# ygina/sidekick

Measured on AMD Instinct MI355X. Metric: quACK encode identifiers/s (device-resident), u32 ids, threshold t=32, higher is better.
Workload: dtype u32; 1 GPU; encode 1e+09 u32 ids per GPU at t=32, device-resident; ids_per_gpu=1000000000, global_ids=1000000000, threshold=32, bits=32, seed=0x5eed0002, parallelism=shard1, collectives=single

## Files before the change

### sidekick_amd/csrc/api.hip

```cpp
#include <string.h>

#include <algorithm>
#include <chrono>
#include <thread>
#include <vector>

#include "ctx.h"
#include "field.h"

using namespace qk;

#pragma clang diagnostic ignored "-Wunused-value"
#pragma clang diagnostic ignored "-Wunused-result"

namespace qk {

QK_WARM_KERNEL(api)

hipStream_t pick_stream(qk_ctx *ctx, void *stream) {
    (void)ctx;
    return (hipStream_t)stream;
}

int scratch_acquire(qk_ctx *ctx, hipStream_t s) {
// ... 551 lines not shown
    if (!ctx) return QK_E_INVAL;
    std::lock_guard<std::mutex> g(ctx->mu);
    ctx->profiling = on != 0;
    return QK_OK;
}

int qk_ctx_kernel_stats(qk_ctx *ctx, double *total_ms, uint64_t *launches) {
    if (!ctx || !total_ms || !launches) return QK_E_INVAL;
    std::lock_guard<std::mutex> g(ctx->mu);
    double tot = 0;
    uint64_t cnt = 0;
    int rc = QK_OK;
    for (auto &pr : ctx->prof_pending) {
        if (hipEventSynchronize(pr.second) != hipSuccess) rc = QK_E_HIP;
        float ms = 0;
        if (hipEventElapsedTime(&ms, pr.first, pr.second) == hipSuccess) { tot += ms; ++cnt; }
        ctx->ev_pool.push_back(pr.first);
        ctx->ev_pool.push_back(pr.second);
    }
    ctx->prof_pending.clear();
    *total_ms = tot;
    *launches = cnt;
    return rc;
}

int qk_ctx_trim(qk_ctx *ctx) {
    if (!ctx) return QK_E_INVAL;
    std::lock_guard<std::mutex> g(ctx->mu);
    if (ctx->retired.empty()) return QK_OK;
    QK_HIP_TRY(hipSetDevice(ctx->device));
    int rc = QK_OK;
    for (void *r : ctx->retired)
        if (hipFree(r) != hipSuccess) rc = QK_E_HIP;
    ctx->retired.clear();
    return rc;
}

int qk_ctx_set_grid(qk_ctx *ctx, uint32_t blocks) {
    if (!ctx) return QK_E_INVAL;
    ctx->grid_override = blocks;
    return QK_OK;
}

int qk_ctx_set_knob(qk_ctx *ctx, const char *name, int64_t value) {
    if (!ctx || !name) return QK_E_INVAL;
    struct K {
        const char *name;
        int qk_knobs::*field;
        int64_t lo, hi;
    };
    static const K table[] = {
        {"grid_mult", &qk_knobs::grid_mult, 1, 8},
        {"enc_dyn", &qk_knobs::enc_dyn, 0, 1},
        {"u32_basis", &qk_knobs::u32_basis, 0, 1},
        {"flow_hist", &qk_knobs::flow_hist, 0, 1 << 20},
        {"flow_byslot", &qk_knobs::flow_byslot, 0, 2},
        {"root_test", &qk_knobs::root_test, 0, 2},
        {"comm_fault", &qk_knobs::comm_fault, 0, 1 << 20},
        {"comm_delay_ms", &qk_knobs::comm_delay_ms, 0, 600000},
        {"rt_karg", &qk_knobs::rt_karg, 0, 1},
    };
    for (const K &k : table)
        if (strcmp(k.name, name) == 0) {
            if (value < k.lo || value > k.hi) return QK_E_INVAL;
            std::lock_guard<std::mutex> g(ctx->mu);
            ctx->knobs.*(k.field) = (int)value;
            return QK_OK;
        }
    return QK_E_INVAL;
}

__global__ void k_clock_probe(uint64_t *out, uint64_t ticks) {
    const uint64_t c0 = __builtin_amdgcn_s_memtime(), r0 = __builtin_amdgcn_s_memrealtime();
    uint64_t c1, r1;
    do {
        __builtin_amdgcn_s_sleep(32);
        c1 = __builtin_amdgcn_s_memtime();
        r1 = __builtin_amdgcn_s_memrealtime();
    } while (r1 - r0 < ticks);
    if (threadIdx.x == 0) {
        out[0] = c1 - c0;
        out[1] = r1 - r0;
    }
}

int qk_clock_probe(qk_ctx *ctx, uint32_t microseconds, uint64_t *d_out, void *stream) {
    if (!ctx || !d_out || !microseconds || microseconds > 10000000u) return QK_E_INVAL;
    if (!is_device_ptr(d_out)) return QK_E_INVAL;
    QK_HIP_TRY(hipSetDevice(ctx->device));
    hipLaunchKernelGGL(k_clock_probe, dim3(1), dim3(64), 0, (hipStream_t)stream, d_out, (uint64_t)microseconds * 100);
    QK_HIP_TRY(hipGetLastError());
    return QK_OK;
}

int qk_host_alloc(size_t bytes, void **out) {
    if (!out) return QK_E_INVAL;
    if (hipHostMalloc(out, bytes, hipHostMallocDefault) != hipSuccess) { *out = nullptr; return QK_E_NOMEM; }
    return QK_OK;
}
int qk_host_free(void *p) {
    if (p && hipHostFree(p) != hipSuccess) return QK_E_HIP;
    return QK_OK;
}

int qk_u32_encode_device_async(qk_ctx *ctx, const uint32_t *d_ids, size_t n, uint32_t t, uint64_t *d_partial,
                               void *stream) {
    if (!ctx || !d_partial || (n && !d_ids)) return QK_E_INVAL;
// ... 157 lines not shown
```

### sidekick_amd/csrc/bsgs.h

```cpp
#pragma once
#include <hip/hip_runtime.h>
#include <stdint.h>

#include "basis32.h"
#include "field.h"

namespace qk {
namespace bsgs {

constexpr int BLOCK = 256;
constexpr int WAVES = BLOCK / 64;

__device__ __forceinline__ uint64_t shfl_xor_u64(uint64_t v, int m) {
    const uint32_t lo = __shfl_xor((int)(uint32_t)v, m, 64);
    const uint32_t hi = __shfl_xor((int)(uint32_t)(v >> 32), m, 64);
    return ((uint64_t)hi << 32) | lo;
}

#define QK_MAC4V(P0, P1, P2, P3)                                                                       \
    "v_mad_u64_u32 %0, " P0 ", %8, %9, %0\n\t"                                                         \
    "v_mad_u64_u32 %1, " P1 ", %8, %10, %1\n\t"                                                        \
    "v_mad_u64_u32 %2, " P2 ", %8, %11, %2\n\t"                                                        \
    "v_mad_u64_u32 %3, " P3 ", %8, %12, %3\n\t"                                                        \
    "v_addc_co_u32_e64 %4, " P0 ", %4, 0, " P0 "\n\t"                                                  \
    "v_addc_co_u32_e64 %5, " P1 ", %5, 0, " P1 "\n\t"                                                  \
    "v_addc_co_u32_e64 %6, " P2 ", %6, 0, " P2 "\n\t"                                                  \
    "v_addc_co_u32_e64 %7, " P3 ", %7, 0, " P3
#define QK_MAC4S(P0, P1, P2, P3, T)                                                                       \
    "v_mad_u64_u32 %0, " P0 ", %8, %9, %0\n\t"                                                         \
    "v_mad_u64_u32 %1, " P1 ", %8, %10, %1\n\t"                                                        \
    "v_mad_u64_u32 %2, " P2 ", %8, %11, %2\n\t"                                                        \
    "v_mad_u64_u32 %3, " P3 ", %8, %12, %3\n\t"                                                        \
    "s_bcnt1_i32_b64 " T ", " P0 "\n\ts_add_u32 %4, %4, " T "\n\t"                                          \
    "s_bcnt1_i32_b64 " T ", " P1 "\n\ts_add_u32 %5, %5, " T "\n\t"                                          \
    "s_bcnt1_i32_b64 " T ", " P2 "\n\ts_add_u32 %6, %6, " T "\n\t"                                          \
    "s_bcnt1_i32_b64 " T ", " P3 "\n\ts_add_u32 %7, %7, " T
#define QK_ADD4V(P0, P1, P2, P3)                                                                       \
    "v_add_co_u32_e64 %0, " P0 ", %0, %8\n\t"                                                          \
    "v_add_co_u32_e64 %1, " P1 ", %1, %9\n\t"                                                          \
    "v_add_co_u32_e64 %2, " P2 ", %2, %10\n\t"                                                         \
    "v_add_co_u32_e64 %3, " P3 ", %3, %11\n\t"                                                         \
    "v_addc_co_u32_e64 %4, " P0 ", %4, 0, " P0 "\n\t"                                                  \
    "v_addc_co_u32_e64 %5, " P1 ", %5, 0, " P1 "\n\t"                                                  \
    "v_addc_co_u32_e64 %6, " P2 ", %6, 0, " P2 "\n\t"                                                  \
    "v_addc_co_u32_e64 %7, " P3 ", %7, 0, " P3
#define QK_ADD4S(P0, P1, P2, P3, T)                                                                       \
    "v_add_co_u32_e64 %0, " P0 ", %0, %8\n\t"                                                          \
    "v_add_co_u32_e64 %1, " P1 ", %1, %9\n\t"                                                          \
    "v_add_co_u32_e64 %2, " P2 ", %2, %10\n\t"                                                         \
    "v_add_co_u32_e64 %3, " P3 ", %3, %11\n\t"                                                         \
    "s_bcnt1_i32_b64 " T ", " P0 "\n\ts_add_u32 %4, %4, " T "\n\t"                                          \
    "s_bcnt1_i32_b64 " T ", " P1 "\n\ts_add_u32 %5, %5, " T "\n\t"                                          \
    "s_bcnt1_i32_b64 " T ", " P2 "\n\ts_add_u32 %6, %6, " T "\n\t"                                          \
    "s_bcnt1_i32_b64 " T ", " P3 "\n\ts_add_u32 %7, %7, " T
#define QK_SET0 "s[40:41]", "s[42:43]", "s[44:45]", "s[46:47]"
#define QK_SET1 "s[48:49]", "s[50:51]", "s[52:53]", "s[54:55]"
#define QK_SET0T QK_SET0, "s56"
// ... 91 lines not shown
                                      uint32_t b0, uint32_t b1) {
    uint64_t k0, k1;
    asm("v_mad_u64_u32 %0, %4, %6, %7, %0\n\t"
        "v_mad_u64_u32 %1, %5, %6, %8, %1\n\t"
        "s_nop 0\n\t"
        "v_addc_co_u32_e64 %2, %4, %2, 0, %4\n\t"
        "v_addc_co_u32_e64 %3, %5, %3, 0, %5"
        : "+v"(a0), "+v"(a1), "+v"(c0), "+v"(c1), "=&s"(k0), "=&s"(k1)
        : "v"(A), "v"(b0), "v"(b1));
}
__device__ __forceinline__ void add2v(uint32_t &l0, uint32_t &l1, uint32_t &c0, uint32_t &c1, uint32_t b0,
                                      uint32_t b1) {
    uint64_t k0, k1;
    asm("v_add_co_u32_e64 %0, %4, %0, %6\n\t"
        "v_add_co_u32_e64 %1, %5, %1, %7\n\t"
        "s_nop 0\n\t"
        "v_addc_co_u32_e64 %2, %4, %2, 0, %4\n\t"
        "v_addc_co_u32_e64 %3, %5, %3, 0, %5"
        : "+v"(l0), "+v"(l1), "+v"(c0), "+v"(c1), "=&s"(k0), "=&s"(k1)
        : "v"(b0), "v"(b1));
}

#define QK_ROW4M(P0, P1, P2, P3)                                                                       \
    "v_mad_u64_u32 %0, " P0 ", %4, 1, %0\n\t"                                                          \
    "v_mad_u64_u32 %1, " P1 ", %5, 1, %1\n\t"                                                          \
    "v_mad_u64_u32 %2, " P2 ", %6, 1, %2\n\t"                                                          \
    "v_mad_u64_u32 %3, " P3 ", %7, 1, %3"
template <int SET>
__device__ __forceinline__ void row4m(uint64_t &a0, uint64_t &a1, uint64_t &a2, uint64_t &a3, uint32_t b0,
                                      uint32_t b1, uint32_t b2, uint32_t b3) {
    if constexpr (SET == 0)
        asm volatile(QK_EXPAND(QK_ROW4M, QK_SET0)
            : "+v"(a0), "+v"(a1), "+v"(a2), "+v"(a3)
            : "v"(b0), "v"(b1), "v"(b2), "v"(b3)
            : QK_CLOB0);
    else
        asm volatile(QK_EXPAND(QK_ROW4M, QK_SET1)
            : "+v"(a0), "+v"(a1), "+v"(a2), "+v"(a3)
            : "v"(b0), "v"(b1), "v"(b2), "v"(b3)
            : QK_CLOB1);
}
__device__ __forceinline__ void row2m(uint64_t &a0, uint64_t &a1, uint32_t b0, uint32_t b1) {
    uint64_t k0, k1;
    asm("v_mad_u64_u32 %0, %2, %4, 1, %0\n\t"
        "v_mad_u64_u32 %1, %3, %5, 1, %1"
        : "+v"(a0), "+v"(a1), "=&s"(k0), "=&s"(k1)
        : "v"(b0), "v"(b1));
}

template <int NB_, int NA_, int SG_, int ROW0_ = 1, int FOLD_ = 1, bool PAIR_ = false, bool OFF_ = false,
          int XC_ = 0, bool TREE_ = false, int PRIO_ = 0>
struct Cfg {
    static constexpr bool BASIS = false;
    static constexpr int PRIO = PRIO_;
    static constexpr int NB = NB_, NA = NA_, SG = SG_, ROW0 = ROW0_, FOLD = FOLD_, XC = XC_;
    static constexpr bool TREE = TREE_;
    static_assert(!TREE_ || (!OFF_ && FOLD_ == 1), "product-tree babies: plain passes, min-tracked folds");
    static constexpr bool PAIR = PAIR_, OFF = OFF_;
    static_assert(OFF_ || (XC_ & 1) == 0, "only an offset pass reads x^base");
    static_assert(!XC_ || FOLD_ == 1, "the x^base cache goes with min-tracked folds");
    static constexpr int ROWS = OFF_ ? NA_ : NA_ - 1;
    static constexpr int ROW1 = OFF_ ? 0 : 1;
    static_assert(NB % 2 == 0 && (NA >= 2 || (OFF_ && NA == 1)), "NB even, NA >= 2 (1: offset pass)");
    static_assert(!OFF_ || FOLD_ == 1, "offset passes use min-tracked folds");
};
template <int PRIO_>
struct CfgBasis : Cfg<8, 4, 8, 1, 1, false, false, 0, false, PRIO_> {
    static constexpr bool BASIS = true;
    static_assert(PRIO_ == 0 || PRIO_ == 4, "basis form: no priority change, or the product's two levels");
};

template <int NB, int NA, int ROWS = NA - 1>
struct Acc {
    uint32_t lo0[NB];
    uint32_t c0[NB];
    uint64_t r0[NB];
    uint64_t m[ROWS][NB];
    uint32_t c[ROWS][NB];
};

template <class C>
__host__ __device__ constexpr bool scalar_group(int row, int b) {
    return b / 4 * 4 + 4 <= C::NB && (row > 0 || C::ROW0 == 0 || C::OFF) && row * (C::NB / 4) + b / 4 < C::SG;
}

template <class MUL>
__device__ __forceinline__ uint32_t pow_uniform(uint32_t xn, uint32_t q, MUL mul) {
    uint32_t r = 0, sq = xn;
    bool have = false;
    for (;;) {
        if (q & 1) {
            r = have ? mul(r, sq) : sq;
            have = true;
        }
        q >>= 1;
        if (!q) break;
        sq = mul(sq, sq);
    }
    return r;
}

#define QK_LP(D, DH, Y, X)                                                                             \
    "v_mad_u64_u32 v[" #D ":" #DH "], s[58:59], " Y ", " X ", 0\n\t"                                   \
    "v_mad_u64_u32 v[6:7], s[58:59], v" #DH ", 5, v[" #D ":" #DH "]\n\t"                               \
    "v_mad_u64_u32 v[" #D ":" #DH "], s[58:59], v7, 5, v[" #D ":" #DH "]\n\t"
#define QK_BT1 QK_LP(8, 9, "v28", "%[id]")
#define QK_BT2 QK_LP(28, 29, "v30", "%[id]") QK_BT1
#define QK_BT3 QK_LP(30, 31, "v32", "%[id]") QK_BT2
#define QK_BT4 QK_LP(32, 33, "v34", "%[id]") QK_BT3
#define QK_BT5 QK_LP(34, 35, "v36", "%[id]") QK_BT4
#define QK_BT6 QK_LP(36, 37, "v38", "%[id]") QK_BT5
#define QK_BABIES4 QK_LP(30, 31, "%[id]", "%[id]") QK_BT2
#define QK_BABIES6 QK_LP(34, 35, "%[id]", "%[id]") QK_BT4
#define QK_BABIES8 QK_LP(38, 39, "%[id]", "%[id]") QK_BT6
#define QK_BMIN4 "v_min3_u32 v9, v30, v28, v8\n\t"
#define QK_BMIN6 QK_BMIN4 "v_min3_u32 v9, v9, v34, v32\n\t"
#define QK_BMIN8 QK_BMIN6 "v_min3_u32 v9, v9, v38, v36\n\t"
#define QK_BOUT4 "=&{v30}"(B[1]), "=&{v28}"(B[2]), "=&{v8}"(B[3])
#define QK_BOUT6 "=&{v34}"(B[1]), "=&{v32}"(B[2]), "=&{v30}"(B[3]), "=&{v28}"(B[4]), "=&{v8}"(B[5])
#define QK_BOUT8                                                                                       \
    "=&{v38}"(B[1]), "=&{v36}"(B[2]), "=&{v34}"(B[3]), "=&{v32}"(B[4]), "=&{v30}"(B[5]), "=&{v28}"(B[6]), \
// ... 26 lines not shown
#define QK_GOUT2 QK_GOUT1, "=&{v12}"(G[1])
#define QK_GOUT3 QK_GOUT2, "=&{v14}"(G[2])
#define QK_GOUT4 QK_GOUT3, "=&{v16}"(G[3])
#define QK_GOUT5 QK_GOUT4, "=&{v18}"(G[4])
#define QK_GOUT6 QK_GOUT5, "=&{v20}"(G[5])
#define QK_GOUT7 QK_GOUT6, "=&{v22}"(G[6])
#define QK_GOUT8 QK_GOUT7, "=&{v24}"(G[7])
#define QK_GOUT9 QK_GOUT8, "=&{v26}"(G[8])
#define QK_GCLOB0
#define QK_GCLOB1 , "v11"
#define QK_GCLOB2 QK_GCLOB1, "v13"
#define QK_GCLOB3 QK_GCLOB2, "v15"
#define QK_GCLOB4 QK_GCLOB3, "v17"
#define QK_GCLOB5 QK_GCLOB4, "v19"
#define QK_GCLOB6 QK_GCLOB5, "v21"
#define QK_GCLOB7 QK_GCLOB6, "v23"
#define QK_GCLOB8 QK_GCLOB7, "v25"
#define QK_GCLOB9 QK_GCLOB8, "v27"

template <int NB, int NG>
struct LazyChain {
    static constexpr bool fused = false;
};
#define QK_CHAIN(NB, NG)                                                                               \
    template <>                                                                                        \
    struct LazyChain<NB, NG> {                                                                         \
        static constexpr bool fused = true;                                                            \
        static __device__ __forceinline__ uint32_t run(uint32_t id, uint32_t (&B)[NB],                 \
                                                       uint32_t (&G)[NG ? NG : 1]) {                   \
            uint32_t mn;                                                                               \
            (void)G;                                                                                   \
            asm(QK_BABIES##NB QK_GIANTS##NG QK_BMIN##NB QK_GMIN##NG                                    \
                : "=&{v9}"(mn), QK_BOUT##NB QK_GOUT##NG                                                \
                : [id] "v"(id)                                                                         \
                : "v6", "v7", QK_BCLOB##NB QK_GCLOB##NG, "s58", "s59");                                \
            return mn;                                                                                 \
        }                                                                                              \
    };
#define QK_CHAINS(NB)                                                                                  \
    QK_CHAIN(NB, 0) QK_CHAIN(NB, 1) QK_CHAIN(NB, 2) QK_CHAIN(NB, 3) QK_CHAIN(NB, 4) QK_CHAIN(NB, 5)    \
    QK_CHAIN(NB, 6) QK_CHAIN(NB, 7) QK_CHAIN(NB, 8) QK_CHAIN(NB, 9)
QK_CHAINS(4)
QK_CHAINS(6)
QK_CHAINS(8)

#define QK_BASIS_CHAIN                                                                                 \
    QK_LP(8, 9, "%[id]", "%[id]")                                                                      \
    QK_LP(10, 11, "v8", "%[id]")                                                                       \
    QK_LP(12, 13, "v10", "v10")                                                                        \
    QK_LP(14, 15, "v12", "v8")                                                                         \
    QK_LP(16, 17, "v12", "v12")                                                                        \
    QK_LP(18, 19, "v14", "v14")                                                                        \
    QK_LP(20, 21, "v16", "%[id]")                                                                      \
    QK_LP(22, 23, "v16", "v10")                                                                        \
    "v_min3_u32 v9, v8, v10, v12\n\t"                                                                  \
    "v_min3_u32 v9, v9, v14, v16\n\t"                                                                  \
    "v_min3_u32 v9, v9, v18, v20\n\t"                                                                  \
    "v_min_u32_e32 v9, v9, v22\n\t"
constexpr bool basis_chain_is(const uint8_t (&t)[3 * basis32::NP]) {
    for (int i = 0; i < basis32::NP; ++i)
        if (basis32::CHAIN[i].power != t[3 * i] || basis32::CHAIN[i].left != t[3 * i + 1] ||
            basis32::CHAIN[i].right != t[3 * i + 2])
            return false;
    return true;
}
static_assert(basis_chain_is({2, 1, 1, 3, 2, 1, 6, 3, 3, 8, 6, 2, 12, 6, 6, 16, 8, 8, 13, 12, 1, 15, 12, 3}),
              "QK_BASIS_CHAIN is basis32::CHAIN written out");
__device__ __forceinline__ uint32_t basis_chain(uint32_t id, uint32_t (&V)[basis32::NE]) {
    uint32_t mn;
    V[0] = id;
    asm(QK_BASIS_CHAIN
        : "=&{v9}"(mn), "=&{v8}"(V[1]), "=&{v10}"(V[2]), "=&{v12}"(V[3]), "=&{v14}"(V[4]), "=&{v16}"(V[5]),
          "=&{v18}"(V[6]), "=&{v20}"(V[7]), "=&{v22}"(V[8])
        : [id] "v"(id)
        : "v6", "v7", "v11", "v13", "v15", "v17", "v19", "v21", "v23", "s58", "s59");
    return mn;
}

constexpr uint32_t WRAP_BELOW = 25u;
template <class C>
__device__ __forceinline__ uint32_t powers(uint32_t id, uint32_t (&B)[C::NB], uint32_t (&A)[C::ROWS],
                                           uint32_t base = 0, uint32_t xb = 0, uint32_t *xnext = nullptr) {
    constexpr int NB = C::NB, NA = C::NA;
    B[0] = id;
    if constexpr (C::OFF) {
        uint32_t mn = 0xFFFFFFFFu;
        if constexpr (LazyChain<NB, 0>::fused) {
            uint32_t G[1];
            mn = LazyChain<NB, 0>::run(id, B, G);
        } else {
#pragma unroll
            for (int b = 1; b < NB; ++b) B[b] = mulfold32_min(B[b - 1], B[0], mn);
        }
        const uint32_t xn = B[NB - 1];
        if constexpr (C::XC & 1) A[0] = xb;
        else A[0] = pow_uniform(xn, base / NB, [&](uint32_t u, uint32_t v) { return mulfold32_min(u, v, mn); });
#pragma unroll
        for (int a = 1; a < NA; ++a) A[a] = mulfold32_min(A[a - 1], xn, mn);
        if constexpr ((C::XC & 2) != 0) *xnext = mulfold32_min(A[NA - 1], xn, mn);
        return mn;
    } else if constexpr (C::FOLD == 0) {
        uint32_t wrapped = 0;
#pragma unroll
        for (int b = 1; b < NB; ++b) B[b] = mulfold32_fast(B[b - 1], B[0], wrapped);
        A[0] = B[NB - 1];
#pragma unroll
        for (int a = 1; a < NA - 1; ++a) A[a] = mulfold32_fast(A[a - 1], A[0], wrapped);
        return wrapped ? 0u : 0xFFFFFFFFu;
    } else {
        constexpr int NG = NA - 2 + ((C::XC & 2) != 0 ? 1 : 0);
        if constexpr (!C::TREE && LazyChain<NB, NG>::fused) {
            uint32_t G[NG ? NG : 1];
            const uint32_t mn = LazyChain<NB, NG>::run(id, B, G);
            A[0] = B[NB - 1];
#pragma unroll
            for (int a = 1; a < NA - 1; ++a) A[a] = G[a - 1];
            if constexpr ((C::XC & 2) != 0) *xnext = G[NA - 2];
            return mn;
        }
        uint32_t mn = 0xFFFFFFFFu;
        if constexpr (C::TREE) {
#pragma unroll
            for (int b = 1; b < NB; ++b) {
                const int h = 1 << (31 - __builtin_clz((unsigned)(b + 1) - 1u));
                B[b] = (b + 1) == 2 * h ? mulfold32_min(B[h - 1], B[h - 1], mn)
                                        : mulfold32_min(B[h - 1], B[b - h], mn);
            }
        } else {
#pragma unroll
// ... 91 lines not shown
        if constexpr (NB % 4 == 2)
            mac2v(S.m[a][NB - 2], S.m[a][NB - 1], S.c[a][NB - 2], S.c[a][NB - 1], A[a], B[NB - 2], B[NB - 1]);
    }
    if constexpr (C::PRIO == 7) {
        __builtin_amdgcn_s_setprio(1);
        row0();
    }
}

template <class C, int G>
__device__ __forceinline__ void basis_direct4(Acc<8, 4, 3> &S, const uint32_t (&V)[basis32::NE]) {
    constexpr int i = 4 * G;
    row4m<G % 2>(S.r0[i], S.r0[i + 1], S.r0[i + 2], S.r0[i + 3], V[basis32::direct_v(i)],
                 V[basis32::direct_v(i + 1)], V[basis32::direct_v(i + 2)], V[basis32::direct_v(i + 3)]);
}
template <class C, int G>
__device__ __forceinline__ void basis_mac4(Acc<8, 4, 3> &S, const uint32_t (&V)[basis32::NE]) {
    constexpr int i = 4 * G, a = i / 8, b = i % 8;
    static_assert(scalar_group<C>(a + 1, b), "basis form: pair MACs are scalar-counted");
    mac4ps<G % 2>(S.m[a][b], S.m[a][b + 1], S.m[a][b + 2], S.m[a][b + 3], S.c[a][b], S.c[a][b + 1], S.c[a][b + 2],
                  S.c[a][b + 3], V[basis32::mac_l(i)], V[basis32::mac_r(i)], V[basis32::mac_l(i + 1)],
                  V[basis32::mac_r(i + 1)], V[basis32::mac_l(i + 2)], V[basis32::mac_r(i + 2)],
                  V[basis32::mac_l(i + 3)], V[basis32::mac_r(i + 3)]);
}
template <class C>
__device__ __forceinline__ void accumulate_basis(Acc<8, 4, 3> &S, const uint32_t (&V)[basis32::NE]) {
    static_assert(basis32::ND == 8 && basis32::NM == 24, "two direct groups, six pair groups");
    basis_direct4<C, 0>(S, V);
    basis_direct4<C, 1>(S, V);
    if constexpr (C::PRIO == 4) __builtin_amdgcn_s_setprio(2);
    basis_mac4<C, 0>(S, V);
    basis_mac4<C, 1>(S, V);
    basis_mac4<C, 2>(S, V);
    basis_mac4<C, 3>(S, V);
    basis_mac4<C, 4>(S, V);
    basis_mac4<C, 5>(S, V);
}
constexpr int basis_slot_power(int a, int b) {
    return a == 0 ? basis32::DIRECT[b] : basis32::MAC[(a - 1) * 8 + b];
}

template <class C> __device__ __forceinline__ void prio_enter() {
    if constexpr (C::PRIO == 1 || C::PRIO == 4 || C::PRIO == 5) __builtin_amdgcn_s_setprio(1);
    if constexpr (C::PRIO == 6) __builtin_amdgcn_s_setprio(3);
    if constexpr (C::PRIO == 7) __builtin_amdgcn_s_setprio(2);
    if constexpr (C::PRIO == 2) __builtin_amdgcn_s_setprio(0);
}
template <class C> __device__ __forceinline__ void prio_exit() {
    if constexpr (C::PRIO == 1 || C::PRIO >= 3) __builtin_amdgcn_s_setprio(0);
    if constexpr (C::PRIO == 2) __builtin_amdgcn_s_setprio(1);
}

template <class C>
__device__ __forceinline__ void one(Acc<C::NB, C::NA, C::ROWS> &S, uint32_t id, uint32_t base = 0, uint32_t xb = 0,
                                    uint32_t *xnext = nullptr) {
    if constexpr (C::BASIS) {
        uint32_t V[basis32::NE];
        const uint32_t mn = basis_chain(id, V);
        prio_enter<C>();
        if constexpr (C::PRIO != 0) __builtin_amdgcn_sched_barrier(0);
        const bool w = mn < WRAP_BELOW;
        if (__builtin_expect(__any(w), 0)) {
            if (w) basis32::chain_exact(id, V);
        }
        accumulate_basis<C>(S, V);
        prio_exit<C>();
        return;
    }
    uint32_t B[C::NB], A[C::ROWS];
    const uint32_t mn = powers<C>(id, B, A, base, xb, xnext);
    prio_enter<C>();
    if constexpr (C::PRIO != 0) __builtin_amdgcn_sched_barrier(0);
    const bool w = mn < WRAP_BELOW;
    if (__builtin_expect(__any(w), 0)) {
        if (w) powers_exact<C>(B, A, base, xb, xnext);
    }
    accumulate<C>(S, B, A);
    prio_exit<C>();
}

template <class C>
__device__ __forceinline__ void two(Acc<C::NB, C::NA, C::ROWS> &S, uint32_t id0, uint32_t id1) {
    static_assert(!C::OFF, "pairs: plain passes only");
    uint32_t B0[C::NB], A0[C::ROWS], B1[C::NB], A1[C::ROWS];
    const bool w0 = powers<C>(id0, B0, A0) < WRAP_BELOW;
    const bool w1 = powers<C>(id1, B1, A1) < WRAP_BELOW;
    if (__builtin_expect(__any(w0 | w1), 0)) {
        if (w0) powers_exact<C>(B0, A0);
        if (w1) powers_exact<C>(B1, A1);
    }
    prio_enter<C>();
    accumulate<C>(S, B0, A0);
    accumulate<C>(S, B1, A1);
    prio_exit<C>();
}

template <class C>
__device__ __forceinline__ void four(Acc<C::NB, C::NA, C::ROWS> &S, uint4 w, uint32_t base,
                                     uint4 xb = make_uint4(0, 0, 0, 0), uint4 *xn = nullptr) {
    if constexpr (C::PAIR) {
        two<C>(S, w.x, w.y);
        two<C>(S, w.z, w.w);
    } else {
        uint4 t = make_uint4(0, 0, 0, 0);
        one<C>(S, w.x, base, xb.x, &t.x);
        one<C>(S, w.y, base, xb.y, &t.y);
        one<C>(S, w.z, base, xb.z, &t.z);
        one<C>(S, w.w, base, xb.w, &t.w);
        if constexpr ((C::XC & 2) != 0) *xn = t;
    }
}

template <class C, class Out>
__device__ __forceinline__ void finish(const Acc<C::NB, C::NA, C::ROWS> &S, uint32_t T, Out out,
                                       uint32_t tid = threadIdx.x) {
    constexpr int NB = C::NB, NA = C::NA;
    __shared__ uint64_t sm[WAVES * NB * NA];
    const int lane = tid & 63, wave = tid >> 6;
#pragma unroll
    for (int a = 0; a < NA; ++a) {
#pragma unroll
        for (int b = 0; b < NB; ++b) {
            const bool sc = scalar_group<C>(a, b);
            const uint32_t c = C::OFF ? S.c[a][b] : a == 0 ? S.c0[b] : S.c[a - C::ROW1][b];
            const uint32_t cl = sc ? (lane == 0 ? c : 0u) : c;
            uint64_t x;
            if (C::OFF) {
                x = (uint64_t)fold64_32(S.m[a][b]) + fold64_32((uint64_t)cl * 25u);
            } else if (a == 0) {
                if constexpr (C::ROW0 == 1) x = S.r0[b];
                else x = (uint64_t)S.lo0[b] + (uint64_t)cl * 5u;
            } else {
                x = (uint64_t)fold64_32(S.m[a - C::ROW1][b]) + fold64_32((uint64_t)cl * 25u);
            }
            x = fold64_32(x);
#pragma unroll
            for (int off = 32; off >= 1; off >>= 1) x += shfl_xor_u64(x, off);
            const int m = C::BASIS ? basis_slot_power(a, b) - 1 : a * NB + b;
            if (lane == 0) sm[wave * (NB * NA) + m] = x;
        }
    }
    __syncthreads();
    for (uint32_t m = tid; m < T; m += BLOCK) {
        uint64_t s = 0;
#pragma unroll
        for (int w = 0; w < WAVES; ++w) s += sm[w * (NB * NA) + m];
        out(m, s);
    }
}

template <class C>
__device__ __forceinline__ void clear(Acc<C::NB, C::NA, C::ROWS> &S) {
#pragma unroll
    for (int b = 0; b < C::NB; ++b) {
        S.lo0[b] = 0;
        S.c0[b] = 0;
        S.r0[b] = 0;
#pragma unroll
        for (int a = 0; a < C::ROWS; ++a) { S.m[a][b] = 0; S.c[a][b] = 0; }
    }
}

template <class C, class Out>
__device__ __forceinline__ void body_gen(const uint32_t *__restrict__ ids, uint64_t n, uint32_t head, uint32_t T,
                                         uint64_t gtid, uint64_t nthr, Out out, uint32_t base = 0,
                                         const uint32_t *xin = nullptr,
                                         uint32_t *xout = nullptr) {
    constexpr bool XI = (C::XC & 1) != 0, XO = (C::XC & 2) != 0;
    Acc<C::NB, C::NA, C::ROWS> S;
    clear<C>(S);
    const uint64_t gbase64 = gtid - threadIdx.x;
    const uint32_t gb_lo = (uint32_t)__builtin_amdgcn_readfirstlane((int)(uint32_t)gbase64);
    const uint32_t gb_hi = (uint32_t)__builtin_amdgcn_readfirstlane((int)(uint32_t)(gbase64 >> 32));
    const uint32_t wave_s = (uint32_t)__builtin_amdgcn_readfirstlane((int)(threadIdx.x >> 6));
    const uint64_t h = head < n ? head : n;
    const uint64_t nbody = (n - h) >> 2;
    const uint4 *__restrict__ v = reinterpret_cast<const uint4 *>(ids + h);
    const uint32_t iters = gtid < nbody ? (uint32_t)((nbody - gtid + nthr - 1) / nthr) : 0u;
    const uint32_t tmax = (uint32_t)__builtin_amdgcn_readfirstlane(iters);
    const uint32_t tmin = (uint32_t)__builtin_amdgcn_readlane((int)iters, 63);
    const uint4 *__restrict__ p = v + gtid;
    const uint4 *pc = XI ? reinterpret_cast<const uint4 *>(xin + h) + gtid : nullptr;
    uint4 *po = XO ? reinterpret_cast<uint4 *>(xout + h) + gtid : nullptr;
    const uint4 *const vend = v + nbody;
    uint4 nxt = make_uint4(0, 0, 0, 0), nxc = make_uint4(0, 0, 0, 0), xo = make_uint4(0, 0, 0, 0);
    if (p < vend) {
        nxt = *p;
        if constexpr (XI) nxc = *pc;
    }
    uint32_t it = 0;
    for (; it + 1 < tmin; ++it) {
        const uint4 w = nxt, c = nxc;
        p += nthr;
        nxt = *p;
        if constexpr (XI) {
            pc += nthr;
            nxc = *pc;
        }
        four<C>(S, w, base, c, &xo);
        if constexpr (XO) {
            *po = xo;
            po += nthr;
        }
    }
    for (; it < tmax; ++it) {
        const uint4 w = nxt, c = nxc;
        const bool cur = p < vend;
        p += nthr;
        nxt = make_uint4(0, 0, 0, 0);
        if (p < vend) nxt = *p;
        if constexpr (XI) {
            pc += nthr;
            if (p < vend) nxc = *pc;
        }
        four<C>(S, w, base, c, &xo);
        if constexpr (XO) {
            if (cur) *po = xo;
            po += nthr;
        }
        (void)cur;
    }
    const uint64_t tail0 = h + (nbody << 2);
    const uint32_t tid = wave_s * 64u + __lane_id();
// ... 24 lines not shown
}

#ifndef QK_DYN_CH
#define QK_DYN_CH 16
#endif
constexpr int DYN_CH = QK_DYN_CH;
constexpr uint32_t DYN_GROUPS = DYN_CH * 64;

__device__ __forceinline__ uint64_t claim_chunk(unsigned long long *ctr, uint64_t cbase) {
    uint32_t lo, hi;
    asm volatile("v_mov_b32_e32 v6, 1\n\t"
                 "v_mov_b32_e32 v7, 0\n\t"
                 "s_mov_b64 s[58:59], exec\n\t"
                 "s_mov_b64 exec, 1\n\t"
                 "global_atomic_add_x2 v[6:7], v7, v[6:7], %[ctr] sc0\n\t"
                 "s_mov_b64 exec, s[58:59]\n\t"
                 "s_waitcnt vmcnt(0)\n\t"
                 "v_readfirstlane_b32 %[lo], v6\n\t"
                 "v_readfirstlane_b32 %[hi], v7"
                 : [lo] "=s"(lo), [hi] "=s"(hi)
                 : [ctr] "s"(ctr)
                 : "v6", "v7", "s58", "s59", "memory");
    return (((uint64_t)hi << 32) | lo) - cbase;
}

typedef uint32_t u32x4_t __attribute__((ext_vector_type(4)));
__device__ __forceinline__ __amdgpu_buffer_rsrc_t chunk_rsrc(const char *vb, uint64_t g) {
    return __builtin_amdgcn_make_buffer_rsrc(const_cast<char *>(vb + g * 16u), 0, (int)(DYN_GROUPS * 16u),
                                             0x00020000);
}
__device__ __forceinline__ uint4 chunk_group(__amdgpu_buffer_rsrc_t rs, uint32_t slot, uint32_t j) {
    const u32x4_t w = __builtin_amdgcn_raw_buffer_load_b128(rs, (int)slot, (int)(j * 1024u), 0);
    return make_uint4(w.x, w.y, w.z, w.w);
}

constexpr int DYN_NCTR = 8;
constexpr int DYN_CTR_STRIDE = 544;
struct DynArgs {
    unsigned long long *ctr;
    uint64_t region;
    uint64_t base[DYN_NCTR];
};
__host__ __device__ inline uint64_t dyn_region_len(uint64_t nchunks, uint64_t region, uint32_t k) {
    const uint64_t lo = (uint64_t)k * region;
    return lo >= nchunks ? 0 : (nchunks - lo < region ? nchunks - lo : region);
}

template <class C>
__device__ __forceinline__ void body_dyn(const uint32_t *__restrict__ ids, uint64_t n, uint32_t head, uint32_t T,
                                         uint64_t *__restrict__ partials, const DynArgs &da) {
    static_assert(!C::OFF && C::XC == 0, "dynamic chunks: plain single-pass configurations");
    Acc<C::NB, C::NA, C::ROWS> S;
    clear<C>(S);
    const uint32_t wave_s = (uint32_t)__builtin_amdgcn_readfirstlane((int)(threadIdx.x >> 6));
    const uint64_t h = head < n ? head : n;
    const uint64_t nbody = (n - h) >> 2;
    const uint64_t nchunks = nbody / DYN_GROUPS;
    const char *vb = reinterpret_cast<const char *>(ids + h);
    const uint32_t slot = __lane_id() * 16u;
    constexpr uint64_t NONE = ~0ull;
    uint32_t k = blockIdx.x % (uint32_t)DYN_NCTR, failed = 0;
    bool rest_mine = false;
    auto claim = [&]() -> uint64_t {
        while (failed < (uint32_t)DYN_NCTR) {
            const uint64_t idx = claim_chunk(da.ctr + (size_t)k * DYN_CTR_STRIDE, da.base[k]);
            const uint64_t len = dyn_region_len(nchunks, da.region, k);
            if (idx < len) return (uint64_t)k * da.region + idx;
            if (k == 0 && idx == len) rest_mine = true;
            k = k + 1 == (uint32_t)DYN_NCTR ? 0u : k + 1;
            ++failed;
        }
        return NONE;
    };
    uint4 nxt = make_uint4(0, 0, 0, 0);
    uint64_t cur = claim();
    __amdgpu_buffer_rsrc_t rs = chunk_rsrc(vb, 0);
    if (cur != NONE) {
        rs = chunk_rsrc(vb, cur * DYN_GROUPS);
        nxt = chunk_group(rs, slot, 0);
    }
    while (cur != NONE) {
        const uint64_t next = claim();
        for (uint32_t j = 1; j < (uint32_t)DYN_CH; ++j) {
            const uint4 w = nxt;
            nxt = chunk_group(rs, slot, j);
            four<C>(S, w, 0);
        }
        const uint4 w = nxt;
        if (next != NONE) {
            rs = chunk_rsrc(vb, next * DYN_GROUPS);
            nxt = chunk_group(rs, slot, 0);
        }
        four<C>(S, w, 0);
        cur = next;
    }
    if (rest_mine) {
        const uint32_t lane = __lane_id();
        const uint32_t rest = (uint32_t)(nbody - nchunks * DYN_GROUPS);
        rs = chunk_rsrc(vb, nchunks * DYN_GROUPS);
        nxt = make_uint4(0, 0, 0, 0);
        if (lane < rest) nxt = chunk_group(rs, slot, 0);
        for (uint32_t j = 0; j * 64u < rest; ++j) {
            const uint4 w = nxt;
            nxt = make_uint4(0, 0, 0, 0);
            if ((j + 1) * 64u + lane < rest) nxt = chunk_group(rs, slot, j + 1);
            four<C>(S, w, 0);
// ... 13 lines not shown
```

### sidekick_amd/csrc/encode.hip

```cpp
#include <algorithm>
#include <type_traits>
#include <utility>

#include "ctx.h"
#include "field.h"
#include "bsgs.h"
#include "bsgs64.h"

#ifndef QK_BSGS_SG_T32
#define QK_BSGS_SG_T32 8
#endif
#ifndef QK_BSGS_ROW0
#define QK_BSGS_ROW0 1
#endif
#ifndef QK_BSGS_FOLD
#define QK_BSGS_FOLD 1
#endif

namespace qk {

QK_WARM_KERNEL(encode)

using bsgs::BLOCK;
using bsgs::WAVES;
using bsgs::shfl_xor_u64;


template <int K>
__device__ __forceinline__ void chain32(uint64_t (&acc)[K], uint32_t start, uint32_t step) {
    const uint32_t step5 = times5_32(step);
    uint64_t t = start;
#pragma unroll
    for (int k = 0; k < K; ++k) {
        acc[k] += t;
        if (k + 1 < K) t = tstep32p(t, step, step5, 0u);
    }
}

template <int K>
__device__ __forceinline__ void chain32x4(uint64_t (&acc)[K], uint4 w) {
    const uint32_t x0 = canon32(w.x), x1 = canon32(w.y), x2 = canon32(w.z), x3 = canon32(w.w);
    const uint32_t f0 = times5_32(x0), f1 = times5_32(x1), f2 = times5_32(x2), f3 = times5_32(x3);
    uint64_t t0 = x0, t1 = x1, t2 = x2, t3 = x3;
#pragma unroll
    for (int k = 0; k < K; ++k) {
        acc[k] += t0;
        acc[k] += t1;
        acc[k] += t2;
        acc[k] += t3;
        if (k + 1 < K) {
            t0 = tstep32p(t0, x0, f0, 0u);
            t1 = tstep32p(t1, x1, f1, 0u);
            t2 = tstep32p(t2, x2, f2, 0u);
            t3 = tstep32p(t3, x3, f3, 0u);
        }
    }
}

template <int NB, int NA, int SG, int PRIO = 1>
__global__ __launch_bounds__(BLOCK, (NB * NA == 32 ? 5 : NB * NA > 64 ? 2 : NB * NA > 40 ? 3 : 4)) void k_encode_u32_bsgs(const uint32_t *__restrict__ ids,
                                                                                  uint64_t n, uint32_t head,
                                                                                  uint32_t T,
                                                                                  uint64_t *__restrict__ partials) {
    bsgs::body<bsgs::Cfg<NB, NA, SG, QK_BSGS_ROW0, QK_BSGS_FOLD, false, false, 0, false, PRIO ? 4 : 0>>(ids, n, head,
                                                                                                        T, partials);
}

template <int NB, int NA, int SG, int PRIO = 1>
__global__ __launch_bounds__(BLOCK, (NB * NA == 32 ? 5 : NB * NA > 64 ? 2 : NB * NA > 40 ? 3 : 4)) void k_encode_u32_bsgs_dyn(
    const uint32_t *__restrict__ ids, uint64_t n, uint32_t head, uint32_t T, uint64_t *__restrict__ partials,
    const bsgs::DynArgs da) {
    bsgs::body_dyn<bsgs::Cfg<NB, NA, SG, QK_BSGS_ROW0, QK_BSGS_FOLD, false, false, 0, false, PRIO ? 4 : 0>>(
        ids, n, head, T, partials, da);
}

template <int PRIO = 1>
__global__ __launch_bounds__(BLOCK, 5) void k_encode_u32_basis(const uint32_t *__restrict__ ids, uint64_t n,
                                                              uint32_t head, uint32_t T,
                                                              uint64_t *__restrict__ partials) {
    bsgs::body<bsgs::CfgBasis<PRIO ? 4 : 0>>(ids, n, head, T, partials);
}
template <int PRIO = 1>
__global__ __launch_bounds__(BLOCK, 5) void k_encode_u32_basis_dyn(const uint32_t *__restrict__ ids, uint64_t n,
                                                                  uint32_t head, uint32_t T,
                                                                  uint64_t *__restrict__ partials,
                                                                  const bsgs::DynArgs da) {
    bsgs::body_dyn<bsgs::CfgBasis<PRIO ? 4 : 0>>(ids, n, head, T, partials, da);
}

template <int SG, int PRIO = 1>
__global__ __launch_bounds__(BLOCK, 2) void k_encode_u32_bsgs_x80(const uint32_t *__restrict__ ids, uint64_t n,
                                                                 uint32_t head, uint32_t T,
                                                                 uint64_t *__restrict__ partials,
                                                                 const uint32_t *xin,
                                                                 uint32_t *xout) {
    (void)xin;
    bsgs::body<bsgs::Cfg<8, 10, SG, 1, 1, false, false, 2, false, PRIO ? 4 : 0>>(ids, n, head, T, partials, 0, nullptr,
                                                                                 xout);
}

template <int NA, int SG, int XC = 0, int PRIO = 1>
__global__ __launch_bounds__(BLOCK, (NA > 6 ? 2 : NA > 5 ? 3 : 4)) void k_encode_u32_bsgs_off(
    const uint32_t *__restrict__ ids, uint64_t n, uint32_t head, uint32_t T, uint32_t base,
    uint64_t *__restrict__ partials, const uint32_t *xin, uint32_t *xout) {
    bsgs::body<bsgs::Cfg<8, NA, SG, 1, 1, false, true, XC, false, PRIO ? 4 : 0>>(ids, n, head, T, partials, base, xin,
                                                                                 xout);
}

template <int G>
__device__ __forceinline__ void group_powers32(uint32_t x, int j, uint32_t &start, uint32_t &step) {
    uint32_t b = x, r = 1;
    const uint32_t e = (uint32_t)j + 1;
#pragma unroll
    for (int bit = 0; (1 << bit) <= G; ++bit) {
        const uint32_t rb = mul32_lazy(r, b);
        r = ((e >> bit) & 1) ? rb : r;
        if ((1 << bit) < G) b = mul32_lazy(b, b);
    }
    start = r;
    step = canon32(b);
}

template <int G, int K, typename Fold>
__device__ __forceinline__ void block_store(const uint64_t (&acc)[K], uint32_t T, uint64_t *partials,
                                            uint64_t *sm, Fold fold) {
    const int lane = threadIdx.x & 63, wave = threadIdx.x >> 6;
#pragma unroll
    for (int k = 0; k < K; ++k) {
        uint64_t v = fold(acc[k]);
#pragma unroll
        for (int off = 32; off >= G; off >>= 1) v += shfl_xor_u64(v, off);
        if (lane < G) sm[wave * (G * K) + lane + k * G] = v;
    }
    __syncthreads();
    for (uint32_t m = threadIdx.x; m < T; m += BLOCK) {
        uint64_t s = 0;
#pragma unroll
        for (int w = 0; w < WAVES; ++w) s += sm[w * (G * K) + m];
        partials[(size_t)m * gridDim.x + blockIdx.x] = s;
    }
// ... 560 lines not shown
        K = k;
        if ((uint32_t)k >= kneed) break;
    }
    return K;
}

template <int KMAX, class KG1, class KGN, int... Gs, class F>
static int enc_chain(uint32_t T, ints<Gs...> gs, F &&gk) {
    int G = 1;
    while ((T + G - 1) / G > (uint32_t)KMAX) G *= 2;
    const uint32_t kneed = (T + G - 1) / G;
    return with_int(G, gs, QK_E_THRESHOLD, [&](auto g) {
        using KS = std::conditional_t<decltype(g)::value == 1, KG1, KGN>;
        return with_int(pick_k(kneed, KS{}), KS{}, QK_E_THRESHOLD, [&](auto k) { return gk(g, k); });
    });
}

#define QK_U32_SHAPES(X)           \
    X(5, 8, 4, 2, 1)               \
    X(9, 12, 4, 3, 3)              \
    X(13, 16, 4, 4, 4)             \
    X(17, 20, 4, 5, 5)             \
    X(21, 24, 4, 6, 6)             \
    X(25, 28, 4, 7, 7)             \
    X(29, 30, 6, 5, 5)             \
    X(31, 32, 8, 4, QK_BSGS_SG_T32) \
    X(33, 36, 6, 6, 6)             \
    X(37, 40, 8, 5, 10)            \
    X(41, 42, 6, 7, 7)             \
    X(43, 48, 8, 6, 12)            \
    X(49, 56, 8, 7, 14)            \
    X(57, 64, 8, 8, 16)            \
    X(65, 72, 8, 9, 14)            \
    X(73, 80, 8, 10, 16)

static int enc32(qk_ctx *ctx, const uint32_t *ids, size_t n, uint32_t T, uint64_t *out, int acc, hipStream_t s) {
    if (T == 0 || T > QK_MAX_THRESHOLD) return QK_E_THRESHOLD;
    const uintptr_t a = (uintptr_t)ids;
    if (a & 3) return QK_E_INVAL;
    const uint32_t head = (uint32_t)(((16 - (a & 15)) & 15) / 4);
    if (n >= (1ull << 40)) return QK_E_INVAL;
    const uint64_t min_grid = ctx->grid_override ? ctx->grid_override : (uint64_t)ctx->num_cus;
    const bool sc_ok = n / (4ull * BLOCK * min_grid) < (1ull << 24) - 2;
    const bool dyn = ctx->knobs.enc_dyn != 0 && n < (1ull << 32);
#define QK_BSGS_STATIC(NB_, NA_, G_)                                                                      \
    run_encode(ctx, k_encode_u32_bsgs<NB_, NA_, G_, 1>, NB_ * NA_, ids, n, head, T, (n + 3) / 4, BLOCK, out, acc, s, \
               NB_ * NA_ > 48 ? 1 : 0)
#define QK_BSGS(NB_, NA_, G_)                                                                             \
    (dyn ? run_encode_dyn(ctx, k_encode_u32_bsgs_dyn<NB_, NA_, G_, 1>, NB_ * NA_, ids, n, head, T, out, acc, s) \
         : QK_BSGS_STATIC(NB_, NA_, G_))
#define QK_BSGS_ROW(LO_, HI_, NB_, NA_, G_) \
    if (T >= LO_ && T <= HI_) return QK_BSGS(NB_, NA_, G_);
    if (sc_ok) {
        if (T >= 31 && T <= 32 && ctx->knobs.u32_basis != 0)
            return dyn ? run_encode_dyn(ctx, k_encode_u32_basis_dyn<1>, 32, ids, n, head, T, out, acc, s)
                       : run_encode(ctx, k_encode_u32_basis<1>, 32, ids, n, head, T, (n + 3) / 4, BLOCK, out, acc, s,
                                    0);
        QK_U32_SHAPES(QK_BSGS_ROW)
        if (T > 80) return enc_passes(ctx, ids, n, head, T, out, acc, s);
    } else {
        if (T >= 9 && T <= 12) return QK_BSGS_STATIC(4, 3, 0);
        if (T >= 13 && T <= 16) return QK_BSGS_STATIC(4, 4, 0);
        if (T >= 17 && T <= 24) return QK_BSGS_STATIC(6, 4, 0);
        if (T >= 25 && T <= 32) return QK_BSGS_STATIC(8, 4, 0);
    }
#undef QK_BSGS_ROW
#undef QK_BSGS
#undef QK_BSGS_STATIC
    return enc_chain<32, K32_G1, K32_GN>(T, ints<1, 2, 4, 8, 16, 32>{}, [&](auto g, auto k) {
        constexpr int G = decltype(g)::value, K = decltype(k)::value;
        if constexpr (G == 1)
            return run_encode(ctx, k_encode_u32_g1<K>, K, ids, n, head, T, (n + 3) / 4, BLOCK, out, acc, s);
        else
            return run_encode(ctx, k_encode_u32_gn<G, K>, G * K, ids, n, head, T, n, BLOCK / G, out, acc, s);
    });
}

static int enc64(qk_ctx *ctx, const uint64_t *ids, size_t n, uint32_t T, uint64_t *out, int acc, hipStream_t s) {
    if (T == 0 || T > QK_MAX_THRESHOLD) return QK_E_THRESHOLD;
    const uintptr_t a = (uintptr_t)ids;
    if (a & 7) return QK_E_INVAL;
    const uint32_t head = (uint32_t)(((16 - (a & 15)) & 15) / 8);
    const uint64_t min_grid64 = ctx->grid_override ? ctx->grid_override : (uint64_t)ctx->num_cus;
    const bool bsgs_ok = n / min_grid64 < (1ull << 30);
    if (T >= 14 && T <= 80 && bsgs_ok) {
        const uint64_t tiles = (n + bsgs64::BLOCK - 1) / bsgs64::BLOCK;
        const int rc4 = with_int(T <= 36 ? (T + 3) / 4 : 0, ints<4, 5, 7, 9>{}, 1, [&](auto na) {
            constexpr int NA = decltype(na)::value;
            return run_encode(ctx, k_encode_u64_bsgs4<NA, 1>, 4 * NA, ids, n, head, T, tiles, 1, out, acc, s);
        });
        if (rc4 <= 0) return rc4;
        return with_int((T + 7) / 8, ints<2, 3, 4, 5, 6, 7, 8, 9, 10>{}, QK_E_THRESHOLD, [&](auto na) {
            constexpr int NA = decltype(na)::value, SG = NA == 10 ? 14 : 16;
            return run_encode(ctx, k_encode_u64_bsgs<NA, SG, 1>, 8 * NA, ids, n, head, T, tiles, 1, out, acc, s);
        });
    }
    if (T > 80 && bsgs_ok) return enc_passes(ctx, ids, n, head, T, out, acc, s);
    return enc_chain<40, K64_G1, K64_GN>(T, ints<1, 2, 4, 8, 16, 32, 64>{}, [&](auto g, auto k) {
        constexpr int G = decltype(g)::value, K = decltype(k)::value;
        if constexpr (G == 1)
            return run_encode(ctx, k_encode_u64_g1<K>, K, ids, n, head, T, (n + 1) / 2, BLOCK, out, acc, s);
        else
            return run_encode(ctx, k_encode_u64_gn<G, K>, G * K, ids, n, head, T, n, BLOCK / G, out, acc, s);
    });
}

int launch_encode_u32(qk_ctx *ctx, const uint32_t *d_ids, size_t n, uint32_t t, uint64_t *d_partial, hipStream_t s) {
    return enc32(ctx, d_ids, n, t, d_partial, 0, s);
}
int launch_encode_u64(qk_ctx *ctx, const uint64_t *d_ids, size_t n, uint32_t t, uint64_t *d_partial, hipStream_t s) {
// ... 13 lines not shown
```

Baseline: 498.9 billion identifiers/s.

## Filter rare wrap-around ids via LDS table and drop per-id min check in basis encode

For the u32 basis encode path at t=31..32, the per-id min-tracking wrap check is replaced by a 16 KiB LDS hash filter of the 61 ids known to need exact handling. Matching ids go through an exact chain and are zeroed; the rest take a lazy chain with no min reduction. This adds a table load per workgroup, LDS lookups per id and a wave vote, and lowers LDS-limited occupancy headroom. The old filterless basis path stays reachable as knob value 2.

Measured after the change: 507.6 billion identifiers/s (median of 6 runs). +1.8%, better.

```diff
diff --git a/sidekick_amd/csrc/api.hip b/sidekick_amd/csrc/api.hip
--- a/sidekick_amd/csrc/api.hip
+++ b/sidekick_amd/csrc/api.hip
@@ -627,7 +627,7 @@
     static const K table[] = {
         {"grid_mult", &qk_knobs::grid_mult, 1, 8},
         {"enc_dyn", &qk_knobs::enc_dyn, 0, 1},
-        {"u32_basis", &qk_knobs::u32_basis, 0, 1},
+        {"u32_basis", &qk_knobs::u32_basis, 0, 2},
         {"flow_hist", &qk_knobs::flow_hist, 0, 1 << 20},
         {"flow_byslot", &qk_knobs::flow_byslot, 0, 2},
         {"root_test", &qk_knobs::root_test, 0, 2},
diff --git a/sidekick_amd/csrc/basis_filter.h b/sidekick_amd/csrc/basis_filter.h
--- /dev/null
+++ b/sidekick_amd/csrc/basis_filter.h
@@ -0,0 +1,70 @@
+#pragma once
+#include <stdint.h>
+
+namespace qk {
+namespace basis_filter {
+
+constexpr int NWRONG = 61;
+constexpr uint32_t WRONG[NWRONG] = {
+    15362091u,   58005635u,   84325748u,   212215109u,  221073260u,  492279886u,  552143393u,
+    622572812u,  639109131u,  957658446u,  998652690u,  1120809293u, 1142778689u, 1248059560u,
+    1373385175u, 1606977228u, 1669389704u, 1793818983u, 1820041303u, 1858945430u, 1974274384u,
+    2039928669u, 2085787571u, 2173567192u, 2255038622u, 2324401375u, 2337445954u, 2436021861u,
+    2474925988u, 2523745003u, 2624686118u, 2625577587u, 2687990063u, 2921582116u, 3046907731u,
+    3152188602u, 3277239954u, 3278929599u, 3365160499u, 3493496785u, 3655858160u, 3672394479u,
+    3742823898u, 3780479003u, 3802687405u, 3828599332u, 3911878746u, 3927921728u, 4073894031u,
+    4082752182u, 4147259949u, 4210641543u, 4236961656u, 4291450497u, 4294836219u, 4294901755u,
+    4294967287u, 4294967288u, 4294967293u, 4294967294u, 4294967295u,
+};
+
+constexpr uint32_t KEY_MASK = 0x3FFCu;
+constexpr int SLOTS = (KEY_MASK >> 2) + 1;
+constexpr uint32_t WINDOW = 0x20004u;
+constexpr uint32_t EMPTY_HIGH = 0x80000000u;
+constexpr uint32_t EMPTY_FLIP = 0x2000u;
+constexpr int USED_SLOTS = 57;
+constexpr uint64_t CANDIDATES = (uint64_t)USED_SLOTS * 36u + (uint64_t)(SLOTS - USED_SLOTS) * 32u;
+
+struct Table {
+    uint32_t e[SLOTS];
+};
+constexpr uint32_t slot_of(uint32_t id) { return (id & KEY_MASK) >> 2; }
+constexpr Table make_table() {
+    Table t{};
+    for (int k = 0; k < SLOTS; ++k) t.e[k] = EMPTY_HIGH | (((uint32_t)k << 2) ^ EMPTY_FLIP);
+    bool used[SLOTS] = {};
+    for (int i = 0; i < NWRONG; ++i) {
+        const uint32_t k = slot_of(WRONG[i]);
+        t.e[k] = used[k] ? (t.e[k] | WRONG[i]) : WRONG[i];
+        used[k] = true;
+    }
+    return t;
+}
+constexpr Table TABLE = make_table();
+
+constexpr bool candidate(const Table &t, uint32_t id) { return (t.e[slot_of(id)] ^ id) < WINDOW; }
+constexpr bool candidate(uint32_t id) { return candidate(TABLE, id); }
+
+constexpr bool list_ok() {
+    for (int i = 1; i < NWRONG; ++i)
+        if (WRONG[i - 1] >= WRONG[i]) return false;
+    return true;
+}
+constexpr bool wrong_are_candidates() {
+    for (int i = 0; i < NWRONG; ++i)
+        if (!candidate(WRONG[i])) return false;
+    return true;
+}
+constexpr int used_slots() {
+    int n = 0;
+    for (int k = 0; k < SLOTS; ++k) n += slot_of(TABLE.e[k]) == (uint32_t)k;
+    return n;
+}
+static_assert(list_ok(), "basis_filter: the wrong ids ascend, none twice");
+static_assert(wrong_are_candidates(), "basis_filter: every wrong id is a candidate (no false negative)");
+static_assert(used_slots() == USED_SLOTS, "basis_filter: slots in use");
+static_assert(!candidate(0u), "basis_filter: id 0 (lanes past their range) takes the fast path");
+static_assert(sizeof(Table) == 16384, "basis_filter: 16 KiB per workgroup, five workgroups per CU");
+
+}
+}
diff --git a/sidekick_amd/csrc/bsgs.h b/sidekick_amd/csrc/bsgs.h
--- a/sidekick_amd/csrc/bsgs.h
+++ b/sidekick_amd/csrc/bsgs.h
@@ -3,6 +3,7 @@
 #include <stdint.h>
 
 #include "basis32.h"
+#include "basis_filter.h"
 #include "field.h"
 
 namespace qk {
@@ -200,6 +201,7 @@
           int XC_ = 0, bool TREE_ = false, int PRIO_ = 0>
 struct Cfg {
     static constexpr bool BASIS = false;
+    static constexpr bool FILT = false;
     static constexpr int PRIO = PRIO_;
     static constexpr int NB = NB_, NA = NA_, SG = SG_, ROW0 = ROW0_, FOLD = FOLD_, XC = XC_;
     static constexpr bool TREE = TREE_;
@@ -212,9 +214,10 @@
     static_assert(NB % 2 == 0 && (NA >= 2 || (OFF_ && NA == 1)), "NB even, NA >= 2 (1: offset pass)");
     static_assert(!OFF_ || FOLD_ == 1, "offset passes use min-tracked folds");
 };
-template <int PRIO_>
+template <int PRIO_, int FILT_ = 1>
 struct CfgBasis : Cfg<8, 4, 8, 1, 1, false, false, 0, false, PRIO_> {
     static constexpr bool BASIS = true;
+    static constexpr bool FILT = FILT_ != 0;
     static_assert(PRIO_ == 0 || PRIO_ == 4, "basis form: no priority change, or the product's two levels");
 };
 
@@ -347,7 +350,9 @@
     QK_LP(16, 17, "v12", "v12")                                                                        \
     QK_LP(18, 19, "v14", "v14")                                                                        \
     QK_LP(20, 21, "v16", "%[id]")                                                                      \
-    QK_LP(22, 23, "v16", "v10")                                                                        \
+    QK_LP(22, 23, "v16", "v10")
+#define QK_BASIS_CHAIN_MIN                                                                             \
+    QK_BASIS_CHAIN                                                                                     \
     "v_min3_u32 v9, v8, v10, v12\n\t"                                                                  \
     "v_min3_u32 v9, v9, v14, v16\n\t"                                                                  \
     "v_min3_u32 v9, v9, v18, v20\n\t"                                                                  \
@@ -361,15 +366,41 @@
 }
 static_assert(basis_chain_is({2, 1, 1, 3, 2, 1, 6, 3, 3, 8, 6, 2, 12, 6, 6, 16, 8, 8, 13, 12, 1, 15, 12, 3}),
               "QK_BASIS_CHAIN is basis32::CHAIN written out");
-__device__ __forceinline__ uint32_t basis_chain(uint32_t id, uint32_t (&V)[basis32::NE]) {
+__device__ __forceinline__ void basis_chain(uint32_t id, uint32_t (&V)[basis32::NE]) {
+    V[0] = id;
+    asm(QK_BASIS_CHAIN
+        : "=&{v8}"(V[1]), "=&{v10}"(V[2]), "=&{v12}"(V[3]), "=&{v14}"(V[4]), "=&{v16}"(V[5]), "=&{v18}"(V[6]),
+          "=&{v20}"(V[7]), "=&{v22}"(V[8])
+        : [id] "v"(id)
+        : "v6", "v7", "v9", "v11", "v13", "v15", "v17", "v19", "v21", "v23", "s58", "s59");
+}
+__device__ __forceinline__ uint32_t basis_chain_min(uint32_t id, uint32_t (&V)[basis32::NE]) {
     uint32_t mn;
     V[0] = id;
-    asm(QK_BASIS_CHAIN
+    asm(QK_BASIS_CHAIN_MIN
         : "=&{v9}"(mn), "=&{v8}"(V[1]), "=&{v10}"(V[2]), "=&{v12}"(V[3]), "=&{v14}"(V[4]), "=&{v16}"(V[5]),
           "=&{v18}"(V[6]), "=&{v20}"(V[7]), "=&{v22}"(V[8])
         : [id] "v"(id)
         : "v6", "v7", "v11", "v13", "v15", "v17", "v19", "v21", "v23", "s58", "s59");
     return mn;
+}
+
+static __device__ const basis_filter::Table FILTER_TABLE = basis_filter::TABLE;
+__device__ __forceinline__ uint32_t *filter_lds() {
+    __shared__ __attribute__((aligned(16))) uint32_t tab[basis_filter::SLOTS];
+    return tab;
+}
+__device__ __forceinline__ void filter_load() {
+    static_assert(basis_filter::SLOTS % (4 * BLOCK) == 0, "whole 16-byte copies per thread");
+    uint4 *dst = reinterpret_cast<uint4 *>(filter_lds());
+    const uint4 *src = reinterpret_cast<const uint4 *>(FILTER_TABLE.e);
+#pragma unroll
+    for (uint32_t i = 0; i < (uint32_t)basis_filter::SLOTS / 4; i += BLOCK) dst[i + threadIdx.x] = src[i + threadIdx.x];
+    __syncthreads();
+}
+__device__ __forceinline__ uint32_t filter_diff(uint32_t id) {
+    const char *tab = reinterpret_cast<const char *>(filter_lds());
+    return *reinterpret_cast<const uint32_t *>(tab + (id & basis_filter::KEY_MASK)) ^ id;
 }
 
 constexpr uint32_t WRAP_BELOW = 25u;
@@ -567,11 +598,38 @@
 }
 
 template <class C>
+__device__ __forceinline__ void basis_one_lazy(Acc<8, 4, 3> &S, uint32_t id) {
+    uint32_t V[basis32::NE];
+    basis_chain(id, V);
+    prio_enter<C>();
+    if constexpr (C::PRIO != 0) __builtin_amdgcn_sched_barrier(0);
+    accumulate_basis<C>(S, V);
+    prio_exit<C>();
+}
+template <class C>
+__device__ __forceinline__ void basis_candidates(Acc<8, 4, 3> &S, uint32_t &id) {
+    const bool c = filter_diff(id) < basis_filter::WINDOW;
+    if (!__any(c)) return;
+    uint32_t V[basis32::NE];
+#pragma unroll
+    for (int i = 0; i < basis32::NE; ++i) V[i] = 0;
+    if (c) basis32::chain_exact(id, V);
+    prio_enter<C>();
+    accumulate_basis<C>(S, V);
+    prio_exit<C>();
+    id = c ? 0u : id;
+}
+
+template <class C>
 __device__ __forceinline__ void one(Acc<C::NB, C::NA, C::ROWS> &S, uint32_t id, uint32_t base = 0, uint32_t xb = 0,
                                     uint32_t *xnext = nullptr) {
-    if constexpr (C::BASIS) {
+    if constexpr (C::BASIS && C::FILT) {
+        basis_candidates<C>(S, id);
+        basis_one_lazy<C>(S, id);
+        return;
+    } else if constexpr (C::BASIS) {
         uint32_t V[basis32::NE];
-        const uint32_t mn = basis_chain(id, V);
+        const uint32_t mn = basis_chain_min(id, V);
         prio_enter<C>();
         if constexpr (C::PRIO != 0) __builtin_amdgcn_sched_barrier(0);
         const bool w = mn < WRAP_BELOW;
@@ -613,7 +671,20 @@
 template <class C>
 __device__ __forceinline__ void four(Acc<C::NB, C::NA, C::ROWS> &S, uint4 w, uint32_t base,
                                      uint4 xb = make_uint4(0, 0, 0, 0), uint4 *xn = nullptr) {
-    if constexpr (C::PAIR) {
+    if constexpr (C::BASIS && C::FILT) {
+        const uint32_t d0 = filter_diff(w.x), d1 = filter_diff(w.y), d2 = filter_diff(w.z), d3 = filter_diff(w.w);
+        const uint32_t d01 = d0 < d1 ? d0 : d1, d23 = d2 < d3 ? d2 : d3;
+        if (__builtin_expect(__any((d01 < d23 ? d01 : d23) < basis_filter::WINDOW), 0)) {
+            basis_candidates<C>(S, w.x);
+            basis_candidates<C>(S, w.y);
+            basis_candidates<C>(S, w.z);
+            basis_candidates<C>(S, w.w);
+        }
+        basis_one_lazy<C>(S, w.x);
+        basis_one_lazy<C>(S, w.y);
+        basis_one_lazy<C>(S, w.z);
+        basis_one_lazy<C>(S, w.w);
+    } else if constexpr (C::PAIR) {
         two<C>(S, w.x, w.y);
         two<C>(S, w.z, w.w);
     } else {
@@ -684,6 +755,7 @@
     constexpr bool XI = (C::XC & 1) != 0, XO = (C::XC & 2) != 0;
     Acc<C::NB, C::NA, C::ROWS> S;
     clear<C>(S);
+    if constexpr (C::BASIS && C::FILT) filter_load();
     const uint64_t gbase64 = gtid - threadIdx.x;
     const uint32_t gb_lo = (uint32_t)__builtin_amdgcn_readfirstlane((int)(uint32_t)gbase64);
     const uint32_t gb_hi = (uint32_t)__builtin_amdgcn_readfirstlane((int)(uint32_t)(gbase64 >> 32));
@@ -814,6 +886,7 @@
     static_assert(!C::OFF && C::XC == 0, "dynamic chunks: plain single-pass configurations");
     Acc<C::NB, C::NA, C::ROWS> S;
     clear<C>(S);
+    if constexpr (C::BASIS && C::FILT) filter_load();
     const uint32_t wave_s = (uint32_t)__builtin_amdgcn_readfirstlane((int)(threadIdx.x >> 6));
     const uint64_t h = head < n ? head : n;
     const uint64_t nbody = (n - h) >> 2;
diff --git a/sidekick_amd/csrc/encode.hip b/sidekick_amd/csrc/encode.hip
--- a/sidekick_amd/csrc/encode.hip
+++ b/sidekick_amd/csrc/encode.hip
@@ -74,18 +74,18 @@
         ids, n, head, T, partials, da);
 }
 
-template <int PRIO = 1>
+template <int PRIO = 1, int FILT = 1>
 __global__ __launch_bounds__(BLOCK, 5) void k_encode_u32_basis(const uint32_t *__restrict__ ids, uint64_t n,
                                                               uint32_t head, uint32_t T,
                                                               uint64_t *__restrict__ partials) {
-    bsgs::body<bsgs::CfgBasis<PRIO ? 4 : 0>>(ids, n, head, T, partials);
-}
-template <int PRIO = 1>
+    bsgs::body<bsgs::CfgBasis<PRIO ? 4 : 0, FILT>>(ids, n, head, T, partials);
+}
+template <int PRIO = 1, int FILT = 1>
 __global__ __launch_bounds__(BLOCK, 5) void k_encode_u32_basis_dyn(const uint32_t *__restrict__ ids, uint64_t n,
                                                                   uint32_t head, uint32_t T,
                                                                   uint64_t *__restrict__ partials,
                                                                   const bsgs::DynArgs da) {
-    bsgs::body_dyn<bsgs::CfgBasis<PRIO ? 4 : 0>>(ids, n, head, T, partials, da);
+    bsgs::body_dyn<bsgs::CfgBasis<PRIO ? 4 : 0, FILT>>(ids, n, head, T, partials, da);
 }
 
 template <int SG, int PRIO = 1>
@@ -752,10 +752,14 @@
 #define QK_BSGS_ROW(LO_, HI_, NB_, NA_, G_) \
     if (T >= LO_ && T <= HI_) return QK_BSGS(NB_, NA_, G_);
     if (sc_ok) {
-        if (T >= 31 && T <= 32 && ctx->knobs.u32_basis != 0)
-            return dyn ? run_encode_dyn(ctx, k_encode_u32_basis_dyn<1>, 32, ids, n, head, T, out, acc, s)
-                       : run_encode(ctx, k_encode_u32_basis<1>, 32, ids, n, head, T, (n + 3) / 4, BLOCK, out, acc, s,
-                                    0);
+        if (T >= 31 && T <= 32 && ctx->knobs.u32_basis == 1)
+            return dyn ? run_encode_dyn(ctx, k_encode_u32_basis_dyn<1, 1>, 32, ids, n, head, T, out, acc, s)
+                       : run_encode(ctx, k_encode_u32_basis<1, 1>, 32, ids, n, head, T, (n + 3) / 4, BLOCK, out, acc,
+                                    s, 0);
+        if (T >= 31 && T <= 32 && ctx->knobs.u32_basis == 2)
+            return dyn ? run_encode_dyn(ctx, k_encode_u32_basis_dyn<1, 0>, 32, ids, n, head, T, out, acc, s)
+                       : run_encode(ctx, k_encode_u32_basis<1, 0>, 32, ids, n, head, T, (n + 3) / 4, BLOCK, out, acc,
+                                    s, 0);
         QK_U32_SHAPES(QK_BSGS_ROW)
         if (T > 80) return enc_passes(ctx, ids, n, head, T, out, acc, s);
     } else {
```
